# ishine/chunkformer

Hardware: AMD Instinct MI355X
Metric: audio-frames/sec (80-dim fbank) through encoder, chunkformer-large chunk=64, 1/2/4/8 GPU (higher is better)
Workload: dtype bf16

## Files before the change

chunkformer_amd/csrc/cfm_kernels.h:

```cpp
#pragma once
#include <hip/hip_runtime.h>
#include <stdint.h>

typedef __bf16 bf16;

#define CFM_HD_INLINE __host__ __device__ __forceinline__

namespace cfm {

int cu_count();

enum { EPI_STORE = 0, EPI_STORE_F32 = 1, EPI_RESID = 2, EPI_QKV = 3, EPI_GLU = 4, EPI_DW2 = 5 };
enum { ACT_NONE = 0, ACT_RELU = 1, ACT_SILU = 2, ACT_SILU_L2E = 3 };

struct EpiArgs {
  const float* bias = nullptr;
  float alpha = 1.f;
  void* out = nullptr;
  void* out2 = nullptr;
  int ldo = 0;
  int row_off = 0;
  float* x = nullptr;
  int ldx = 0;
  const uint8_t* rowmask = nullptr;
  int d = 0;
  int dk = 64;
  int col_group = 0;
  int store_mode = 0;
  int diag = 0;
  int wst = 1;
  int small_tiles = 0;
  int big_min_tiles = 0;
  int wsp_small_div = 1;
  int wsp_small_rows = 32768;
  int f16 = 0;
  const float* dw_w = nullptr;
  const float* dw_b = nullptr;
  int t2n = 0, t3n = 0;
};

int gemm_bf16_wst(int epi, int act, const bf16* A, int lda, const bf16* W, int ldw, int M, int N, int K,
                  const EpiArgs& ep, hipStream_t st);

enum { SITE_QKV = 1, SITE_OPROJ = 2, SITE_PW2 = 4, SITE_FFN2 = 8, SITE_FFN1 = 16, SITE_PW1 = 32, SITE_FE = 64 };

struct Tuning {
  int gemm_diag = 0, gemm_wst = 1, store_mode = 0, col_group = 0;
  int attn_reuse = 1;
  int conv_dot2 = 2;
  int conv_dma = 1;
  int dw2_seg = 4;
  int fe_conv = 6;
  int fe_fuse_dw2 = 1;
  int attn128_var = 1;
  int nt_sites = 8;
  int big_min_tiles = 0;
  int wsp_small_div = 1;
  int wsp_small_rows = 32768;
  int attn_min_chunks = 2;
  void apply(EpiArgs& e, int site = 0) const {
    e.diag = gemm_diag;
    e.big_min_tiles = big_min_tiles;
    e.wsp_small_div = wsp_small_div;
    e.wsp_small_rows = wsp_small_rows;
    e.wst = gemm_wst;
    e.store_mode = (nt_sites & site) ? 2 : store_mode;
    e.col_group = col_group;
  }
};

template <typename T>
int gemm(int epi, int act, const T* A, int lda, const T* W, int ldw, int M, int N, int K, const EpiArgs& ep,
         hipStream_t st);


template <typename T> struct ResidAdd {
  const T* y = nullptr;
  float alpha = 1.f;
  const uint8_t* ymask = nullptr;
  const T* y2 = nullptr;
  float alpha2 = 1.f;
  const uint8_t* ymask2 = nullptr;
  bool defer = false;
};
template <typename T>
int layernorm(float* x, const ResidAdd<T>& ra, int M, int d, const float* w, const float* b, float eps, T* out,
              const uint8_t* rowmask, hipStream_t st);
template <typename T>
int layernorm2(float* x, const ResidAdd<T>& ra, int M, int d, const float* w1, const float* b1, const float* w2,
               const float* b2, float eps, T* out, hipStream_t st);
template <typename T>
int layernorm2_f32(float* x, const ResidAdd<T>& ra, int M, int d, const float* w1, const float* b1, const float* w2,
                   const float* b2, float eps, float* out, hipStream_t st);

template <typename T>
int chunk_attention(const T* q, const T* kv, int kv_rows, const T* P, int p_rows, const float* pos_u,
                    const float* pos_v, const int32_t* desc, int nblk, int H, int dk, T* out, hipStream_t st,
                    int p_ld = 0);

CFM_HD_INLINE int qkv_kv_col(int cc, int which, int dk) { return (cc / dk) * 2 * dk + which * dk + (cc & (dk - 1)); }

int full_attention_bf16(const bf16* q, const bf16* kv, int kv_rows, const bf16* P, int p_rows, const float* pos_u,
                        const float* pos_v, const int32_t* desc, int nutt, int nd, int H, int dk, int t_keys,
                        bf16* out, hipStream_t st, int p_ld);
int chunk_attention_masked_bf16(const bf16* q, const bf16* kv, int kv_rows, const bf16* P, int p_rows,
                                const float* pos_u, const float* pos_v, const int32_t* desc, int n_chunks, int H,
                                int C, int W, bf16* out, hipStream_t st, int diag = 0, int p_ld = 0, int reuse = 1,
                                int min_chunks = 2);
int chunk_attention_masked_f16(const f16* q, const f16* kv, int kv_rows, const f16* P, int p_rows,
                               const float* pos_u, const float* pos_v, const int32_t* desc, int n_chunks, int H,
                               int C, int W, f16* out, hipStream_t st, int diag = 0, int p_ld = 0, int reuse = 1,
                               int min_chunks = 2);

bool attention_a128_eligible(int C, int W, int p_rows, int dk);
int vt_transpose_bf16(const bf16* kv, int kv_rows, int H, bf16* vt, int vt_ld, hipStream_t st);
int chunk_attention_masked_a128(const bf16* q, const bf16* kv, int kv_rows, const bf16* vt, int vt_ld, const bf16* P,
                                int p_rows, int p_ld, const float* pos_u, const float* pos_v, const int32_t* desc,
                                int n_chunks, int H, int C, int W, bf16* out, hipStream_t st, int var = 1);

template <typename T>
int conv_dw_ln_silu(const T* glu, const int32_t* desc, int nblk, int d, const float* wdw_t ,
                    const float* bdw, const float* lnw, const float* lnb, float eps, T* out, hipStream_t st,
                    int dot2 = 1, int dma = 1);

template <typename T>
int frontend_conv0_dw(const float* feats, const float* const* tab, int step, const int32_t* meta, int meta_stride,
                      int nwin, int W,
                      const float* cmvn_mean, const float* cmvn_istd, const float* w0, const float* b0,
                      const float* w1, const float* b1, const float* wpack, const float* wfrag, int d, T* out,
                      hipStream_t st, int var = 1);
constexpr int FE_WPACK = 24;
constexpr int FE2_NFRAG = 23;
template <typename T>
int frontend_dw2(const T* in, int nwin, int T2, int d, const float* w, const float* b, T* out, hipStream_t st,
                 int seg = 4);

template <typename T>
int pos_table(int d, int p_rows, int anchor, T* out, hipStream_t st);
template <typename T>
int att_cache_in(const float* cache, int L, int row_elems, T* kv, hipStream_t st);
template <typename T>
int att_cache_out(const T* kv, int start_row, int L, int row_elems, float* cache, hipStream_t st);
template <typename T>
int att_cache_in_hl(const float* cache , int H, int L, int dk, T* kv, hipStream_t st);
template <typename T>
int att_cache_out_hl(const T* kv, int start_row, int H, int L, int dk, float* cache , hipStream_t st);
template <typename T>
int cnn_cache_in(const float* cache , int d, int lorder, T* glu, hipStream_t st);
template <typename T>
int cnn_cache_out(const T* glu, int start_row, int d, int lorder, float* cache, hipStream_t st);
template <typename T>
int cache_io(bool in, bool hl, float* acache, int H, int L, int dk, T* kv, float* ccache, int d, int lorder, T* glu,
             hipStream_t st);
int masks_from_plan(const int32_t* meta, int n, int C, int L, int R, uint8_t* att, uint8_t* pad, hipStream_t st);
bool ctc_argmax_eligible(int V, int d);
int ctc_argmax_bf16(const float* enc, int M, const bf16* W, const float* bias, int V, int d, int32_t* ids,
// ... 10 lines not shown
```

chunkformer_amd/csrc/conv_module.hip:

```cpp
#include <algorithm>
#include <cstdlib>
#include <type_traits>
#include "cfm_common.h"
#include "cfm_kernels.h"

namespace cfm {

template <typename T, int VPL> struct VecIO;
template <int VPL> struct VecIO<float, VPL> {
  static CFM_DEV void load(const float* p, float (&v)[VPL]) {
#pragma unroll
    for (int e = 0; e < VPL; e += 2) {
      typedef float f2 __attribute__((ext_vector_type(2)));
      const f2 t = *reinterpret_cast<const f2*>(p + e);
      v[e] = t[0]; v[e + 1] = t[1];
    }
  }
  static CFM_DEV void store(float* p, const float (&v)[VPL]) {
#pragma unroll
    for (int e = 0; e < VPL; e += 2) {
      typedef float f2 __attribute__((ext_vector_type(2)));
      *reinterpret_cast<f2*>(p + e) = (f2){v[e], v[e + 1]};
    }
  }
// ... 110 lines not shown
#pragma unroll
  for (int r = 0; r < RW; ++r) {
    if (i0 + r >= nout) break;
    float sum = 0.f;
#pragma unroll
    for (int e = 0; e < VPL; ++e) sum += acc[r][e];
    const float mean = wave_sum(sum) / d;
    float q = 0.f;
#pragma unroll
    for (int e = 0; e < VPL; ++e) { const float t = acc[r][e] - mean; q += t * t; }
    const float rstd = rsqrtf(wave_sum(q) / d + eps);
    bvec o;
#pragma unroll
    for (int e = 0; e < VPL; ++e) o[e] = (bf16)silu_f((acc[r][e] - mean) * rstd * lw[e] + lb[e]);
    *reinterpret_cast<bvec*>(out + (size_t)(out_row0 + i0 + r) * d + c0) = o;
  }
}

typedef __bf16 bf16x2_t __attribute__((ext_vector_type(2)));
typedef _Float16 f16x2_t __attribute__((ext_vector_type(2)));
template <typename E>
CFM_DEV float dot2e(unsigned a, unsigned b, float c) {
  if constexpr (std::is_same<E, f16>::value)
    return __builtin_amdgcn_fdot2(__builtin_bit_cast(f16x2_t, a), __builtin_bit_cast(f16x2_t, b), c, false);
  else
    return __builtin_amdgcn_fdot2_f32_bf16(__builtin_bit_cast(bf16x2_t, a), __builtin_bit_cast(bf16x2_t, b), c, false);
}
template <typename E>
CFM_DEV unsigned pke(float lo, float hi) {
  typedef E e2 __attribute__((ext_vector_type(2)));
  return __builtin_bit_cast(unsigned, (e2){(E)lo, (E)hi});
}
template <int VPL, typename E>
CFM_DEV void conv_dot2_rows(const E* __restrict__ win, int nout, int out_row0, const float* __restrict__ wdw,
                            const float* __restrict__ bdw, const float* __restrict__ lnw,
                            const float* __restrict__ lnb, float eps, E* __restrict__ out, int w, int lane,
                            int win_row0 = 0) {
  constexpr int d = VPL * 64, NW = VPL / 2;
  constexpr int RW = 8;
  typedef E bvec __attribute__((ext_vector_type(VPL)));
  const int i0 = w * RW;
  if (i0 >= nout) return;
  win -= (size_t)win_row0 * d;
  const int c0 = lane * VPL;
  unsigned wp[8][VPL];
#pragma unroll
  for (int p = 0; p < 8; ++p) {
    float lo[VPL], hi[VPL];
    VecIO<float, VPL>::load(wdw + (2 * p) * d + c0, lo);
    if (p < 7) {
      VecIO<float, VPL>::load(wdw + (2 * p + 1) * d + c0, hi);
    } else {
#pragma unroll
      for (int e = 0; e < VPL; ++e) hi[e] = 0.f;
    }
#pragma unroll
    for (int e = 0; e < VPL; ++e) wp[p][e] = pke<E>(lo[e], hi[e]);
  }
  float acc[RW][VPL];
#pragma unroll
  for (int e = 0; e < VPL; ++e) {
    const float bv = bdw[c0 + e];
#pragma unroll
    for (int r = 0; r < RW; ++r) acc[r][e] = bv;
  }
  auto ld = [&](unsigned (&x)[NW], int row) {
    const unsigned* p = reinterpret_cast<const unsigned*>(win + row * d + c0);
    if constexpr (NW == 4) {
      const u32x4 t = *reinterpret_cast<const u32x4*>(p);
      x[0] = t[0]; x[1] = t[1]; x[2] = t[2]; x[3] = t[3];
    } else if constexpr (NW == 2) {
      typedef unsigned u32x2_ __attribute__((ext_vector_type(2)));
      const u32x2_ t = *reinterpret_cast<const u32x2_*>(p);
      x[0] = t[0]; x[1] = t[1];
    } else {
      x[0] = p[0];
    }
  };
  unsigned ra[NW], rb[NW];
  ld(ra, i0);
#pragma unroll
  for (int j = 0; j < RW + 14; ++j) {
    ld(rb, i0 + j + 1);
    unsigned pk[VPL];
#pragma unroll
    for (int k = 0; k < NW; ++k) {
      pk[2 * k] = __builtin_amdgcn_perm(rb[k], ra[k], 0x05040100u);
      pk[2 * k + 1] = __builtin_amdgcn_perm(rb[k], ra[k], 0x07060302u);
    }
#pragma unroll
    for (int r = 0; r < RW; ++r) {
      const int t = j - r;
      if (t >= 0 && t <= 14 && (t & 1) == 0) {
#pragma unroll
        for (int e = 0; e < VPL; ++e) acc[r][e] = dot2e<E>(pk[e], wp[t >> 1][e], acc[r][e]);
      }
    }
#pragma unroll
    for (int k = 0; k < NW; ++k) ra[k] = rb[k];
  }
  float lw[VPL], lb[VPL];
#pragma unroll
  for (int e = 0; e < VPL; ++e) {
    lw[e] = lnw[c0 + e];
    lb[e] = lnb[c0 + e];
  }
#pragma unroll
  for (int r = 0; r < RW; ++r) {
    if (i0 + r >= nout) break;
    float sum = 0.f;
#pragma unroll
    for (int e = 0; e < VPL; ++e) sum += acc[r][e];
    const float mean = wave_sum_dpp(sum) / d;
    float q = 0.f;
#pragma unroll
    for (int e = 0; e < VPL; ++e) { const float t = acc[r][e] - mean; q += t * t; }
    const float rstd = rsqrtf(wave_sum_dpp(q) / d + eps);
    bvec o;
#pragma unroll
    for (int e = 0; e < VPL; ++e) {
      const float y = (acc[r][e] - mean) * rstd * lw[e] + lb[e];
      o[e] = (E)(y * __builtin_amdgcn_rcpf(1.0f + __builtin_amdgcn_exp2f(-1.4426950408889634f * y)));
    }
    __builtin_nontemporal_store(o, reinterpret_cast<bvec*>(out + (size_t)(out_row0 + i0 + r) * d + c0));
  }
}

template <int VPL, typename E>
__global__ __launch_bounds__(512) void conv_dw_ln_silu_dot2_kernel(const E* __restrict__ glu,
                                                                   const int32_t* __restrict__ desc,
                                                                   const float* __restrict__ wdw,
                                                                   const float* __restrict__ bdw,
                                                                   const float* __restrict__ lnw,
                                                                   const float* __restrict__ lnb, float eps,
                                                                   E* __restrict__ out, int dma) {
  constexpr int d = VPL * 64, NW = VPL / 2;
  constexpr int MAXJ = 64 + 15;
  constexpr int RW = 8;
  typedef E bvec __attribute__((ext_vector_type(VPL)));
  __shared__ __attribute__((aligned(16))) E win[MAXJ * d];
  const int tid = threadIdx.x, lane = tid & 63, w = tid >> 6;
  const int32_t* D = desc + (size_t)blockIdx.x * CD_INTS;
  const int out_row0 = D[CD_OUT_ROW0], nout = D[CD_NOUT], src0 = D[CD_SRC_ROW0];
  const int nj = nout + 14;
  const int jlo = max(D[CD_J_LO], 0), jhi = min(D[CD_J_HI], nj);
  constexpr int V8 = d / 8;
  if (VPL == 8 && dma) {
    for (int j = __builtin_amdgcn_readfirstlane(w); j < MAXJ; j += 8) {
      if (j >= jlo && j < jhi)
        __builtin_amdgcn_global_load_lds((const __attribute__((address_space(1))) void*)(glu + (size_t)(src0 + j) * d + lane * 8),
                                         (__attribute__((address_space(3))) void*)(win + j * d), 16, 0, 0);
      else
        *reinterpret_cast<u32x4*>(win + j * d + lane * 8) = (u32x4){0u, 0u, 0u, 0u};
    }
    asm volatile("s_waitcnt vmcnt(0)" ::: "memory");
  } else {
    for (int idx = tid; idx < MAXJ * V8; idx += 512) {
      const int j = idx / V8, v = idx % V8;
// ... 19 lines not shown
  constexpr int HJ = QR + 15;
  __shared__ __attribute__((aligned(16))) E win[HJ * d];
  const int tid = threadIdx.x, lane = tid & 63, w = tid >> 6;
  const int half = blockIdx.y;
  const int32_t* D = desc + (size_t)blockIdx.x * CD_INTS;
  const int out_row0 = D[CD_OUT_ROW0], nout = D[CD_NOUT], src0 = D[CD_SRC_ROW0];
  if (QR * half >= nout) return;
  const int nj = nout + 14;
  const int jlo = max(D[CD_J_LO], 0), jhi = min(D[CD_J_HI], nj);
  const int r0 = QR * half;
  if (VPL == 8) {
    for (int jj = __builtin_amdgcn_readfirstlane(w); jj < HJ; jj += NWV) {
      const int j = r0 + jj;
      if (j >= jlo && j < jhi)
        __builtin_amdgcn_global_load_lds((const __attribute__((address_space(1))) void*)(glu + (size_t)(src0 + j) * d + lane * 8),
                                         (__attribute__((address_space(3))) void*)(win + jj * d), 16, 0, 0);
      else
        *reinterpret_cast<u32x4*>(win + jj * d + lane * 8) = (u32x4){0u, 0u, 0u, 0u};
    }
    asm volatile("s_waitcnt vmcnt(0)" ::: "memory");
  } else {
    constexpr int V8 = d / 8;
    for (int idx = tid; idx < HJ * V8; idx += QR * 8) {
      const int jj = idx / V8, v = idx % V8, j = r0 + jj;
      u32x4 val = (u32x4){0u, 0u, 0u, 0u};
      if (j >= jlo && j < jhi) val = *reinterpret_cast<const u32x4*>(glu + (size_t)(src0 + j) * d + v * 8);
      *reinterpret_cast<u32x4*>(win + jj * d + v * 8) = val;
    }
  }
  __syncthreads();
  conv_dot2_rows<VPL, E>(win, nout, out_row0, wdw, bdw, lnw, lnb, eps, out, NWV * half + w, lane, r0);
}

template <typename T>
int conv_dw_ln_silu(const T* glu, const int32_t* desc, int nblk, int d, const float* wdw_t, const float* bdw,
                    const float* lnw, const float* lnb, float eps, T* out, hipStream_t st, int dot2, int dma) {
  if (nblk <= 0) return 0;
  if constexpr (sizeof(T) == 2) {
    if (dot2 >= 2 && d == 512) {
      if (dot2 == 3)
        hipLaunchKernelGGL((conv_dw_ln_silu_dot2h_kernel<8, 16, T>), dim3(nblk, 4), dim3(128), 0, st, glu, desc, wdw_t, bdw, lnw, lnb, eps, out);
      else
        hipLaunchKernelGGL((conv_dw_ln_silu_dot2h_kernel<8, 32, T>), dim3(nblk, 2), dim3(256), 0, st, glu, desc, wdw_t, bdw, lnw, lnb, eps, out);
      CFM_CHECK_LAUNCH();
      return 0;
    }
    if (dot2) {
      if (d == 128) hipLaunchKernelGGL((conv_dw_ln_silu_dot2_kernel<2, T>), dim3(nblk), dim3(512), 0, st, glu, desc, wdw_t, bdw, lnw, lnb, eps, out, dma);
      else if (d == 256) hipLaunchKernelGGL((conv_dw_ln_silu_dot2_kernel<4, T>), dim3(nblk), dim3(512), 0, st, glu, desc, wdw_t, bdw, lnw, lnb, eps, out, dma);
      else if (d == 512) hipLaunchKernelGGL((conv_dw_ln_silu_dot2_kernel<8, T>), dim3(nblk), dim3(512), 0, st, glu, desc, wdw_t, bdw, lnw, lnb, eps, out, dma);
      else return (int)hipErrorInvalidValue;
      CFM_CHECK_LAUNCH();
      return 0;
    }
    if constexpr (std::is_same<T, bf16>::value) {
      if (d == 128) hipLaunchKernelGGL((conv_dw_ln_silu_lds_kernel<2>), dim3(nblk), dim3(512), 0, st, glu, desc, wdw_t, bdw, lnw, lnb, eps, out);
      else if (d == 256) hipLaunchKernelGGL((conv_dw_ln_silu_lds_kernel<4>), dim3(nblk), dim3(512), 0, st, glu, desc, wdw_t, bdw, lnw, lnb, eps, out);
      else if (d == 512) hipLaunchKernelGGL((conv_dw_ln_silu_lds_kernel<8>), dim3(nblk), dim3(512), 0, st, glu, desc, wdw_t, bdw, lnw, lnb, eps, out);
      else return (int)hipErrorInvalidValue;
      CFM_CHECK_LAUNCH();
      return 0;
    }
  }
  const dim3 grid(nblk, 4);
  if (d == 128) hipLaunchKernelGGL((conv_dw_ln_silu_kernel<T, 2>), grid, dim3(256), 0, st, glu, desc, wdw_t, bdw, lnw, lnb, eps, out);
  else if (d == 256) hipLaunchKernelGGL((conv_dw_ln_silu_kernel<T, 4>), grid, dim3(256), 0, st, glu, desc, wdw_t, bdw, lnw, lnb, eps, out);
  else if (d == 512) hipLaunchKernelGGL((conv_dw_ln_silu_kernel<T, 8>), grid, dim3(256), 0, st, glu, desc, wdw_t, bdw, lnw, lnb, eps, out);
  else return (int)hipErrorInvalidValue;
  CFM_CHECK_LAUNCH();
  return 0;
}

template int conv_dw_ln_silu<float>(const float*, const int32_t*, int, int, const float*, const float*, const float*,
                                    const float*, float, float*, hipStream_t, int, int);
template int conv_dw_ln_silu<bf16>(const bf16*, const int32_t*, int, int, const float*, const float*, const float*,
                                   const float*, float, bf16*, hipStream_t, int, int);
template int conv_dw_ln_silu<f16>(const f16*, const int32_t*, int, int, const float*, const float*, const float*,
                                   const float*, float, f16*, hipStream_t, int, int);

}
```

chunkformer_amd/csrc/model.hip:

```cpp
#include <algorithm>
#include <cmath>
#include <cstdlib>
#include <cstring>
#include <map>
#include <memory>
#include <string>
#include <vector>

#include "../../include/cfm.h"
#include "../../include/cfm_ops.h"
#include "cfm_common.h"
#include "cfm_kernels.h"
#include "plan.h"
#include "status.h"

namespace cfm {

static thread_local std::string g_err;
cfm_status set_error(cfm_status s, const std::string& msg) {
  g_err = msg;
  return s;
}

#define HIPC(x)                                                                               \
// ... 354 lines not shown
                                            tune.attn_reuse, tune.attn_min_chunks);
          else if (w.vt) {
            KCHK(vt_transpose_bf16(w.kv, kv_rows, H, w.vt, w.vt_ld, st));
            r = chunk_attention_masked_a128(w.q, w.kv, kv_rows, w.vt, w.vt_ld, w.P + (size_t)l * d, p_rows, p_ld,
                                            Lw.pu, Lw.pv, attd, aB, H, C, hh[PH_L] + C + hh[PH_R], w.ao, st,
                                            tune.attn128_var);
          }
          else if (!masked && !stream && hh[PH_L] == 0 && hh[PH_R] == 0 && hh[PH_C] == hh[PH_TOUT] &&
                   use_ring_attention && natt == hh[PH_NWIN] * ((hh[PH_TOUT] + 63) / 64))
            r = full_attention_bf16(w.q, w.kv, kv_rows, w.P + (size_t)l * d, p_rows, Lw.pu, Lw.pv, attd, hh[PH_NWIN],
                                    (hh[PH_TOUT] + 63) / 64, H, dk, hh[PH_TOUT], w.ao, st, p_ld);
        }
        if constexpr (std::is_same<T, f16>::value) {
          if (masked && use_ring_attention && dk == 64)
            r = chunk_attention_masked_f16(w.q, w.kv, kv_rows, w.P + (size_t)l * d, p_rows, Lw.pu, Lw.pv, attd, aB, H, C,
                                           hh[PH_L] + C + hh[PH_R], w.ao, st, attn_diag, p_ld, tune.attn_reuse,
                                           tune.attn_min_chunks);
        }
        if (r == -1)
          r = chunk_attention<T>(w.q, w.kv, kv_rows, w.P + (size_t)l * d, p_rows, Lw.pu, Lw.pv, attd, aB,
                                 H, dk, w.ao, st, p_ld);
        KCHK(r);
        prof_end(PC_ATTN, st, pb_);
      }
      { EpiArgs e = E(SITE_OPROJ); e.bias = Lw.b_o; e.out = w.y2; e.ldo = d;
        PROF(PC_OPROJ, gemm<T>(EPI_STORE, ACT_NONE, w.ao, d, (const T*)Lw.wo, d, rB, d, d, e, st)); }
      PROF(PC_LN, layernorm<T>(w.x, resid2(w.y, 0.5f, nullptr, w.y2, 1.f, nullptr), rB, d, Lw.ln_conv_w, Lw.ln_conv_b,
                               eps, w.h, (masked || stream) ? nullptr : rmask, st));
      if (cci && !cfuse_in) PROF(PC_CACHE, cnn_cache_in<T>(cci + l * cnn_ls, d, 7, w.glu, st));
      { EpiArgs e = E(SITE_PW1); e.bias = Lw.b_pw1; e.out = w.glu; e.ldo = d; e.row_off = gluoff;
        PROF(PC_PW1, gemm<T>(EPI_GLU, kSiluPre<T> ? ACT_SILU_L2E : ACT_NONE, w.h, d, (const T*)Lw.pw1, d, rB, 2 * d, d, e, st)); }
      if (cci && cco && !cfuse_out) PROF(PC_CACHE, cnn_cache_out<T>(w.glu, cache_start, d, 7, cco + l * cnn_ls, st));
      PROF(PC_CONV, conv_dw_ln_silu<T>(w.glu, convd, vN, d, Lw.dw_t, Lw.b_dw, Lw.cn_w, Lw.cn_b, eps, w.cv, st,
                                        tune.conv_dot2, tune.conv_dma));
      { EpiArgs e = E(SITE_PW2); e.bias = Lw.b_pw2; e.out = w.y; e.ldo = d;
        PROF(PC_PW2, gemm<T>(EPI_STORE, ACT_NONE, w.cv, d, (const T*)Lw.pw2, d, rN, d, d, e, st)); }
      { ResidAdd<T> r = resid(w.y, 1.f, rmask); r.defer = true;
        PROF(PC_LN, layernorm<T>(w.x, r, rN, d, Lw.ln_ff_w, Lw.ln_ff_b, eps, w.h, nullptr, st)); }
      { const cfm_status fs = ffn(Lw.ff1, Lw.b_ff1, Lw.ff2, Lw.b_ff2, w.y2, rN); if (fs != CFM_OK) return fs; }
      const ResidAdd<T> rf = resid2(w.y, 1.f, rmask, w.y2, 0.5f, nullptr);
      if (l + 1 < nl)
        PROF(PC_LN, layernorm2<T>(w.x, rf, rN, d, Lw.ln_fin_w, Lw.ln_fin_b, layers[l + 1].ln_ffm_w,
                                  layers[l + 1].ln_ffm_b, eps, w.h, st));
      else
        PROF(PC_LN, layernorm2_f32<T>(w.x, rf, rN, d, Lw.ln_fin_w, Lw.ln_fin_b, fe.an_w, fe.an_b, eps, out, st));
      { const cfm_status cs = caches_out(l); if (cs != CFM_OK) return cs; }
    }
    return CFM_OK;
  }

  cfm_status ctc(const float* enc, int rows, float* logp, int32_t* ids, void* ws, size_t wsb,
                 hipStream_t st) const override {
    if (!fe.ctc_w) return set_error(CFM_ERR_ASSERT, "model has no CTC head (vocab == 0)");
    const int d = cfg.d_model, V = cfg.vocab;
    if constexpr (sizeof(T) == 2) {
      if (!logp && ids && fused_ctc_ok()) {
        int r;
        if constexpr (std::is_same<T, bf16>::value)
          PROF(PC_CTC, (r = ctc_argmax_bf16(enc, rows, (const bf16*)fe.ctc_w, fe.ctc_b, V, d, ids, st)) < 0 ? 0 : r);
        else
          PROF(PC_CTC, (r = ctc_argmax_f16(enc, rows, (const f16*)fe.ctc_w, fe.ctc_b, V, d, ids, st)) < 0 ? 0 : r);
        if (r == 0) return CFM_OK;
      }
    }
    if (wsb < ctc_ws_bytes(rows)) return set_error(CFM_ERR_VALUE, "ctc workspace too small");
    float* dst = nullptr;
    { const cfm_status hs = head_logits(enc, rows, logp, ws, st, &dst); if (hs != CFM_OK) return hs; }
    PROF(PC_CTC, log_softmax_rows(dst, rows, V, logp ? 1 : 0, ids, st));
    return CFM_OK;
  }

  cfm_status head_logits(const float* enc, int rows, float* logp, void* ws, hipStream_t st, float** out) const {
    const int d = cfg.d_model, V = cfg.vocab;
    Carver c(ws);
    float* logits = c.take<float>((size_t)rows * V);
    T* a = c.take<T>((size_t)rows * d);
    const T* A;
    if constexpr (sizeof(T) == 4) {
// ... 287 lines not shown
cfm_status cfm_model_create(const cfm_config* cfg, const cfm_tensor_view* weights, int32_t n, int32_t device,
                            cfm_model** out) {
  if (!cfg || !out) return set_error(CFM_ERR_VALUE, "null argument");
  *out = nullptr;
  if (cfg->input_dim != 80) return set_error(CFM_ERR_ASSERT, "front-end kernel supports input_dim == 80");
  if (cfg->d_model != 128 && cfg->d_model != 256 && cfg->d_model != 512)
    return set_error(CFM_ERR_ASSERT, "d_model must be 128, 256 or 512");
  if (cfg->n_heads <= 0 || (cfg->d_model != 64 * cfg->n_heads && cfg->d_model != 128 * cfg->n_heads))
    return set_error(CFM_ERR_ASSERT, "head_dim (d_model / attention_heads) must be 64 or 128");
  if (cfg->ffn_dim % 128) return set_error(CFM_ERR_ASSERT, "ffn_dim must be a multiple of 128");
  if (cfg->kernel_size != 15) return set_error(CFM_ERR_ASSERT, "cnn_module_kernel must be 15");
  if (cfg->num_blocks <= 0 || cfg->vocab < 0) return set_error(CFM_ERR_VALUE, "bad num_blocks / vocab");
  HostW hw;
  for (int i = 0; i < n; ++i) hw.m[weights[i].name] = {weights[i].data, weights[i].numel};
  if (cfg->compute_dtype == CFM_DTYPE_F32) return build_model<float>(*cfg, hw, device, out);
  if (cfg->compute_dtype == CFM_DTYPE_BF16) return build_model<bf16>(*cfg, hw, device, out);
  if (cfg->compute_dtype == CFM_DTYPE_F16) return build_model<f16>(*cfg, hw, device, out);
  return set_error(CFM_ERR_VALUE, "unknown compute dtype");
}

void cfm_model_destroy(cfm_model* m) { delete m; }

cfm_status cfm_model_set_option(cfm_model* m, const char* key, int64_t value) {
  if (!m || !key) return set_error(CFM_ERR_VALUE, "null argument");
  if (!std::strcmp(key, "max_layers")) { m->max_layers = (int)value; return CFM_OK; }
  if (!std::strcmp(key, "fe_group_windows")) { m->fe_group_windows = (int)std::max<int64_t>(0, value); return CFM_OK; }
  if (!std::strcmp(key, "profile")) { m->prof_mask = (uint32_t)value; return CFM_OK; }
  if (!std::strcmp(key, "ring_attention")) { m->use_ring_attention = value != 0; return CFM_OK; }
  if (!std::strcmp(key, "ctc_fused")) { m->use_fused_ctc = value != 0; return CFM_OK; }
  {
    const std::pair<const char*, int*> knobs[] = {
        {"gemm_diag", &m->tune.gemm_diag}, {"gemm_wst", &m->tune.gemm_wst},   {"store_mode", &m->tune.store_mode},
        {"col_group", &m->tune.col_group}, {"attn_reuse", &m->tune.attn_reuse}, {"conv_dot2", &m->tune.conv_dot2},
        {"conv_dma", &m->tune.conv_dma},   {"dw2_seg", &m->tune.dw2_seg},   {"nt_sites", &m->tune.nt_sites},
        {"fe_fuse_dw2", &m->tune.fe_fuse_dw2}, {"fe_conv", &m->tune.fe_conv},
        {"attn128_var", &m->tune.attn128_var},
        {"gemm_big_min", &m->tune.big_min_tiles}, {"wsp_small_div", &m->tune.wsp_small_div},
        {"wsp_small_rows", &m->tune.wsp_small_rows},
        {"attn_min_chunks", &m->tune.attn_min_chunks}};
    for (auto& k : knobs)
      if (!std::strcmp(key, k.first)) { *k.second = (int)value; return CFM_OK; }
  }
  if (!std::strcmp(key, "attn_diag")) { m->attn_diag = (int)value; return CFM_OK; }
  if (!std::strcmp(key, "cache_fuse")) { m->cache_fuse = (int)(value != 0); return CFM_OK; }
  if (!std::strcmp(key, "trim_right")) { m->trim_right = (int)(value != 0); return CFM_OK; }
  if (!std::strcmp(key, "fe_carry")) { m->fe_carry = reinterpret_cast<float*>((intptr_t)value); return CFM_OK; }
  if (!std::strcmp(key, "fe_reuse")) { m->fe_reuse = (int)std::max<int64_t>(0, value); return CFM_OK; }
  if (!std::strcmp(key, "fe_save_from")) { m->fe_save_from = (int)value; return CFM_OK; }
  if (!std::strcmp(key, "profile_reset")) {
    m->prof_collect();
    for (int i = 0; i < PC_N; ++i) { m->prof_ms[i] = 0; m->prof_n[i] = 0; }
    return CFM_OK;
  }
  return set_error(CFM_ERR_VALUE, std::string("unknown option ") + key);
}

size_t cfm_workspace_bytes_masked(const cfm_model* m, int32_t N, int32_t C, int32_t L, int32_t R) {
  if (!m || N <= 0 || C <= 0) return 0;
  int32_t h[PH_HEADER] = {0};
  const int rows = N * C;
  h[PH_KIND] = 1; h[PH_NWIN] = N; h[PH_ROWS] = rows; h[PH_C] = C; h[PH_L] = L; h[PH_R] = R;
  h[PH_W] = (C - 1) * 8 + 15; h[PH_TOUT] = C; h[PH_PROWS] = L + 2 * C + R - 1;
  h[PH_KVROWS] = L + rows + R; h[PH_GLUROWS] = rows + 14;
  return m->ws_bytes(h);
}

// ... 224 lines not shown
```

chunkformer_amd/csrc/norm.hip:

```cpp
#include "cfm_common.h"
#include "cfm_kernels.h"

#ifndef LN_RPW
#define LN_RPW 1
#endif
#ifndef LN2_RPW
#define LN2_RPW 2
#endif
#ifndef LN_Y16
#define LN_Y16 0
#endif

namespace cfm {

template <int VPL>
CFM_DEV void ln_row(float (&v)[VPL], int d, const float* w, const float* b, float eps, int lane) {
  float s = 0.f;
#pragma unroll
  for (int e = 0; e < VPL; ++e) s += v[e];
  const float mean = wave_sum_dpp(s) / d;
  float q = 0.f;
#pragma unroll
  for (int e = 0; e < VPL; ++e) {
    const float t = v[e] - mean;
// ... 116 lines not shown
      }
    }
    ln_row<VPL>(v0, d, w, b, eps, lane);
    ln_row<VPL>(v1, d, w, b, eps, lane);
    if (rowmask) {
#pragma unroll
      for (int e = 0; e < VPL; ++e) {
        if (!rowmask[row0]) v0[e] = 0.f;
        if (!rowmask[row1]) v1[e] = 0.f;
      }
    }
    store_row(out + (size_t)row0 * d + lane * VPL, v0);
    if (row1 != row0) store_row(out + (size_t)row1 * d + lane * VPL, v1);
    return;
  }
  const int row = blockIdx.x * 4 + (threadIdx.x >> 6);
  if (row >= M) return;
  float v[VPL];
  float* xp = x + (size_t)row * d + lane * VPL;
  load_row(xp, v);
  resid_add<T, VPL>(v, xp, ra, row, lane);
  ln_row<VPL>(v, d, w, b, eps, lane);
  if (rowmask && !rowmask[row]) {
#pragma unroll
    for (int e = 0; e < VPL; ++e) v[e] = 0.f;
  }
  store_row(out + (size_t)row * d + lane * VPL, v);
}

template <typename TY, typename TO, int VPL>
__global__ __launch_bounds__(256) void ln2_kernel(float* __restrict__ x, ResidAdd<TY> ra, int M,
                                                  const float* __restrict__ w1, const float* __restrict__ b1,
                                                  const float* __restrict__ w2, const float* __restrict__ b2, float eps,
                                                  TO* __restrict__ out) {
  const int lane = threadIdx.x & 63;
  constexpr int d = VPL * 64;
  if constexpr (LN2_RPW == 2) {
    const int row0 = (blockIdx.x * 4 + (threadIdx.x >> 6)) * 2;
    if (row0 >= M) return;
    const int row1 = row0 + 1 < M ? row0 + 1 : row0;
    float v0[VPL], v1[VPL];
    float* xp0 = x + (size_t)row0 * d + lane * VPL;
    float* xp1 = x + (size_t)row1 * d + lane * VPL;
    load_row(xp0, v0);
    load_row(xp1, v1);
    if (ra.y) {
      resid_terms<TY, VPL>(v0, ra, row0, lane);
      resid_terms<TY, VPL>(v1, ra, row1, lane);
    }
    ln_row<VPL>(v0, d, w1, b1, eps, lane);
    ln_row<VPL>(v1, d, w1, b1, eps, lane);
    store_row(xp0, v0);
    if (row1 != row0) store_row(xp1, v1);
    if (w2) {
      ln_row<VPL>(v0, d, w2, b2, eps, lane);
      ln_row<VPL>(v1, d, w2, b2, eps, lane);
    }
    store_row(out + (size_t)row0 * d + lane * VPL, v0);
    if (row1 != row0) store_row(out + (size_t)row1 * d + lane * VPL, v1);
    return;
  }
  const int row = blockIdx.x * 4 + (threadIdx.x >> 6);
  if (row >= M) return;
  float v[VPL];
  float* xp = x + (size_t)row * d + lane * VPL;
  load_row(xp, v);
  if (ra.y) resid_terms<TY, VPL>(v, ra, row, lane);
  ln_row<VPL>(v, d, w1, b1, eps, lane);
  store_row(xp, v);
  if (w2) ln_row<VPL>(v, d, w2, b2, eps, lane);
  store_row(out + (size_t)row * d + lane * VPL, v);
}

template <typename T>
int layernorm(float* x, const ResidAdd<T>& ra, int M, int d, const float* w, const float* b, float eps, T* out,
              const uint8_t* rowmask, hipStream_t st) {
  if (M <= 0) return 0;
  const int nblk = (M + 4 * LN_RPW - 1) / (4 * LN_RPW);
  if (d == 128) hipLaunchKernelGGL((ln_kernel<T, 2>), dim3(nblk), dim3(256), 0, st, x, ra, M, w, b, eps, out, rowmask);
  else if (d == 256) hipLaunchKernelGGL((ln_kernel<T, 4>), dim3(nblk), dim3(256), 0, st, x, ra, M, w, b, eps, out, rowmask);
  else if (d == 512) hipLaunchKernelGGL((ln_kernel<T, 8>), dim3(nblk), dim3(256), 0, st, x, ra, M, w, b, eps, out, rowmask);
  else return (int)hipErrorInvalidValue;
  CFM_CHECK_LAUNCH();
  return 0;
}

template <typename TY, typename TO>
static int ln2_launch(float* x, const ResidAdd<TY>& ra, int M, int d, const float* w1, const float* b1, const float* w2,
                      const float* b2, float eps, TO* out, hipStream_t st) {
  if (M <= 0) return 0;
  const int nblk = (M + 4 * LN2_RPW - 1) / (4 * LN2_RPW);
  if (d == 128) hipLaunchKernelGGL((ln2_kernel<TY, TO, 2>), dim3(nblk), dim3(256), 0, st, x, ra, M, w1, b1, w2, b2, eps, out);
  else if (d == 256) hipLaunchKernelGGL((ln2_kernel<TY, TO, 4>), dim3(nblk), dim3(256), 0, st, x, ra, M, w1, b1, w2, b2, eps, out);
  else if (d == 512) hipLaunchKernelGGL((ln2_kernel<TY, TO, 8>), dim3(nblk), dim3(256), 0, st, x, ra, M, w1, b1, w2, b2, eps, out);
  else return (int)hipErrorInvalidValue;
  CFM_CHECK_LAUNCH();
  return 0;
}

template <typename T>
int layernorm2(float* x, const ResidAdd<T>& ra, int M, int d, const float* w1, const float* b1, const float* w2,
               const float* b2, float eps, T* out, hipStream_t st) {
  return ln2_launch<T, T>(x, ra, M, d, w1, b1, w2, b2, eps, out, st);
}
template <typename T>
int layernorm2_f32(float* x, const ResidAdd<T>& ra, int M, int d, const float* w1, const float* b1, const float* w2,
                   const float* b2, float eps, float* out, hipStream_t st) {
  return ln2_launch<T, float>(x, ra, M, d, w1, b1, w2, b2, eps, out, st);
}

template int layernorm<float>(float*, const ResidAdd<float>&, int, int, const float*, const float*, float, float*,
                              const uint8_t*, hipStream_t);
template int layernorm<bf16>(float*, const ResidAdd<bf16>&, int, int, const float*, const float*, float, bf16*,
                             const uint8_t*, hipStream_t);
template int layernorm<f16>(float*, const ResidAdd<f16>&, int, int, const float*, const float*, float, f16*,
                             const uint8_t*, hipStream_t);
template int layernorm2<float>(float*, const ResidAdd<float>&, int, int, const float*, const float*, const float*,
                               const float*, float, float*, hipStream_t);
template int layernorm2<bf16>(float*, const ResidAdd<bf16>&, int, int, const float*, const float*, const float*,
                              const float*, float, bf16*, hipStream_t);
template int layernorm2<f16>(float*, const ResidAdd<f16>&, int, int, const float*, const float*, const float*,
                              const float*, float, f16*, hipStream_t);
template int layernorm2_f32<float>(float*, const ResidAdd<float>&, int, int, const float*, const float*, const float*,
                                   const float*, float, float*, hipStream_t);
template int layernorm2_f32<bf16>(float*, const ResidAdd<bf16>&, int, int, const float*, const float*, const float*,
                                  const float*, float, float*, hipStream_t);
template int layernorm2_f32<f16>(float*, const ResidAdd<f16>&, int, int, const float*, const float*, const float*,
                                  const float*, float, float*, hipStream_t);

}
```

Measured before the change: 32.68 million.

## Add persistent double-buffered conv kernel and skip final-layer residual store

Adds a persistent depthwise-conv+LN+SiLU kernel that walks chunk groups per CU with double-buffered LDS staging through global_load_lds, and reuses overlapping halo rows between consecutive chunks. It is selected only when conv_dot2==4, and the default is 2, so it is opt-in through a new conv_blocks knob. Separately, the last layer's layernorm2_f32 now skips writing the normalized residual back to x, which saves one full-width fp32 store that nothing downstream reads. The LN change is on by default, and it is a problem if any later consumer does read x after the final layer.

```diff
diff --git a/chunkformer_amd/csrc/cfm_kernels.h b/chunkformer_amd/csrc/cfm_kernels.h
--- a/chunkformer_amd/csrc/cfm_kernels.h
+++ b/chunkformer_amd/csrc/cfm_kernels.h
@@ -48,6 +48,7 @@
   int gemm_diag = 0, gemm_wst = 1, store_mode = 0, col_group = 0;
   int attn_reuse = 1;
   int conv_dot2 = 2;
+  int conv_blocks = 0;
   int conv_dma = 1;
   int dw2_seg = 4;
   int fe_conv = 6;
@@ -91,7 +92,7 @@
                const float* b2, float eps, T* out, hipStream_t st);
 template <typename T>
 int layernorm2_f32(float* x, const ResidAdd<T>& ra, int M, int d, const float* w1, const float* b1, const float* w2,
-                   const float* b2, float eps, float* out, hipStream_t st);
+                   const float* b2, float eps, float* out, hipStream_t st, bool store_x = true);
 
 template <typename T>
 int chunk_attention(const T* q, const T* kv, int kv_rows, const T* P, int p_rows, const float* pos_u,
@@ -121,7 +122,7 @@
 template <typename T>
 int conv_dw_ln_silu(const T* glu, const int32_t* desc, int nblk, int d, const float* wdw_t ,
                     const float* bdw, const float* lnw, const float* lnb, float eps, T* out, hipStream_t st,
-                    int dot2 = 1, int dma = 1);
+                    int dot2 = 1, int dma = 1, int blocks = 0);
 
 template <typename T>
 int frontend_conv0_dw(const float* feats, const float* const* tab, int step, const int32_t* meta, int meta_stride,
diff --git a/chunkformer_amd/csrc/conv_module.hip b/chunkformer_amd/csrc/conv_module.hip
--- a/chunkformer_amd/csrc/conv_module.hip
+++ b/chunkformer_amd/csrc/conv_module.hip
@@ -166,18 +166,8 @@
   return __builtin_bit_cast(unsigned, (e2){(E)lo, (E)hi});
 }
 template <int VPL, typename E>
-CFM_DEV void conv_dot2_rows(const E* __restrict__ win, int nout, int out_row0, const float* __restrict__ wdw,
-                            const float* __restrict__ bdw, const float* __restrict__ lnw,
-                            const float* __restrict__ lnb, float eps, E* __restrict__ out, int w, int lane,
-                            int win_row0 = 0) {
-  constexpr int d = VPL * 64, NW = VPL / 2;
-  constexpr int RW = 8;
-  typedef E bvec __attribute__((ext_vector_type(VPL)));
-  const int i0 = w * RW;
-  if (i0 >= nout) return;
-  win -= (size_t)win_row0 * d;
-  const int c0 = lane * VPL;
-  unsigned wp[8][VPL];
+CFM_DEV void conv_dot2_taps(const float* __restrict__ wdw, int c0, unsigned (&wp)[8][VPL]) {
+  constexpr int d = VPL * 64;
 #pragma unroll
   for (int p = 0; p < 8; ++p) {
     float lo[VPL], hi[VPL];
@@ -191,10 +181,15 @@
 #pragma unroll
     for (int e = 0; e < VPL; ++e) wp[p][e] = pke<E>(lo[e], hi[e]);
   }
-  float acc[RW][VPL];
+}
+template <int VPL, typename E>
+CFM_DEV void conv_dot2_acc(const E* __restrict__ win, int i0, int c0, const unsigned (&wp)[8][VPL],
+                           const float (&bias)[VPL], float (&acc)[8][VPL]) {
+  constexpr int d = VPL * 64, NW = VPL / 2;
+  constexpr int RW = 8;
 #pragma unroll
   for (int e = 0; e < VPL; ++e) {
-    const float bv = bdw[c0 + e];
+    const float bv = bias[e];
 #pragma unroll
     for (int r = 0; r < RW; ++r) acc[r][e] = bv;
   }
@@ -233,31 +228,61 @@
 #pragma unroll
     for (int k = 0; k < NW; ++k) ra[k] = rb[k];
   }
+}
+template <int VPL, typename E, bool STORE = true>
+CFM_DEV void conv_dot2_finish(float (&acc)[8][VPL], const float (&lw)[VPL], const float (&lb)[VPL], float eps,
+                              int nout, int i0, int out_row0, int c0, E* __restrict__ out) {
+  constexpr int d = VPL * 64;
+  constexpr int RW = 8;
+  typedef E bvec __attribute__((ext_vector_type(VPL)));
+#pragma unroll
+  for (int r = 0; r < RW; ++r) {
+    if (i0 + r >= nout) break;
+    float sum = 0.f;
+#pragma unroll
+    for (int e = 0; e < VPL; ++e) sum += acc[r][e];
+    const float mean = wave_sum_dpp(sum) / d;
+    float q = 0.f;
+#pragma unroll
+    for (int e = 0; e < VPL; ++e) { const float t = acc[r][e] - mean; q += t * t; }
+    const float rstd = rsqrtf(wave_sum_dpp(q) / d + eps);
+    bvec o;
+#pragma unroll
+    for (int e = 0; e < VPL; ++e) {
+      const float y = (acc[r][e] - mean) * rstd * lw[e] + lb[e];
+      o[e] = (E)(y * __builtin_amdgcn_rcpf(1.0f + __builtin_amdgcn_exp2f(-1.4426950408889634f * y)));
+    }
+    if constexpr (STORE)
+      __builtin_nontemporal_store(o, reinterpret_cast<bvec*>(out + (size_t)(out_row0 + i0 + r) * d + c0));
+    else if (o[0] == (E)12345.f)
+      __builtin_nontemporal_store(o, reinterpret_cast<bvec*>(out + (size_t)(out_row0 + i0 + r) * d + c0));
+  }
+}
+template <int VPL, typename E>
+CFM_DEV void conv_dot2_rows(const E* __restrict__ win, int nout, int out_row0, const float* __restrict__ wdw,
+                            const float* __restrict__ bdw, const float* __restrict__ lnw,
+                            const float* __restrict__ lnb, float eps, E* __restrict__ out, int w, int lane,
+                            int win_row0 = 0) {
+  constexpr int d = VPL * 64;
+  constexpr int RW = 8;
+  const int i0 = w * RW;
+  if (i0 >= nout) return;
+  win -= (size_t)win_row0 * d;
+  const int c0 = lane * VPL;
+  unsigned wp[8][VPL];
+  conv_dot2_taps<VPL, E>(wdw, c0, wp);
+  float bias[VPL];
+#pragma unroll
+  for (int e = 0; e < VPL; ++e) bias[e] = bdw[c0 + e];
+  float acc[RW][VPL];
+  conv_dot2_acc<VPL, E>(win, i0, c0, wp, bias, acc);
   float lw[VPL], lb[VPL];
 #pragma unroll
   for (int e = 0; e < VPL; ++e) {
     lw[e] = lnw[c0 + e];
     lb[e] = lnb[c0 + e];
   }
-#pragma unroll
-  for (int r = 0; r < RW; ++r) {
-    if (i0 + r >= nout) break;
-    float sum = 0.f;
-#pragma unroll
-    for (int e = 0; e < VPL; ++e) sum += acc[r][e];
-    const float mean = wave_sum_dpp(sum) / d;
-    float q = 0.f;
-#pragma unroll
-    for (int e = 0; e < VPL; ++e) { const float t = acc[r][e] - mean; q += t * t; }
-    const float rstd = rsqrtf(wave_sum_dpp(q) / d + eps);
-    bvec o;
-#pragma unroll
-    for (int e = 0; e < VPL; ++e) {
-      const float y = (acc[r][e] - mean) * rstd * lw[e] + lb[e];
-      o[e] = (E)(y * __builtin_amdgcn_rcpf(1.0f + __builtin_amdgcn_exp2f(-1.4426950408889634f * y)));
-    }
-    __builtin_nontemporal_store(o, reinterpret_cast<bvec*>(out + (size_t)(out_row0 + i0 + r) * d + c0));
-  }
+  conv_dot2_finish<VPL, E>(acc, lw, lb, eps, nout, i0, out_row0, c0, out);
 }
 
 template <int VPL, typename E>
@@ -343,11 +368,138 @@
   conv_dot2_rows<VPL, E>(win, nout, out_row0, wdw, bdw, lnw, lnb, eps, out, NWV * half + w, lane, r0);
 }
 
+#ifndef CFM_CONV_DIAG
+#define CFM_CONV_DIAG 0
+#endif
+template <typename E>
+__global__ __launch_bounds__(512) void conv_dw_ln_silu_dot2p_kernel(const E* __restrict__ glu,
+                                                                    const int32_t* __restrict__ desc, int nblk,
+                                                                    const float* __restrict__ wdw,
+                                                                    const float* __restrict__ bdw,
+                                                                    const float* __restrict__ lnw,
+                                                                    const float* __restrict__ lnb, float eps,
+                                                                    E* __restrict__ out) {
+  constexpr int VPL = 8, d = 512;
+  constexpr int WJ = 64 + 15;
+  __shared__ __attribute__((aligned(16))) E win[2][WJ * d];
+  const int lane = threadIdx.x & 63, w = __builtin_amdgcn_readfirstlane(threadIdx.x >> 6);
+  const long long G = 8ll * nblk;
+  const int g0 = (int)(G * blockIdx.x / gridDim.x), g1 = (int)(G * (blockIdx.x + 1) / gridDim.x);
+  if (g0 >= g1) return;
+  const int c0 = lane * VPL;
+  unsigned wp[8][VPL];
+  conv_dot2_taps<VPL, E>(wdw, c0, wp);
+  float bias[VPL], lw[VPL], lb[VPL];
+#pragma unroll
+  for (int e = 0; e < VPL; ++e) {
+    bias[e] = bdw[c0 + e];
+    lw[e] = lnw[c0 + e];
+    lb[e] = lnb[c0 + e];
+  }
+  struct It { int out_row0, nout, src0, jlo, jhi, ga, ng; };
+  auto fetch = [&](int s) {
+    const int32_t* D = desc + (size_t)(s >> 3) * CD_INTS;
+    It c;
+    c.out_row0 = D[CD_OUT_ROW0]; c.nout = D[CD_NOUT]; c.src0 = D[CD_SRC_ROW0];
+    c.jlo = max(D[CD_J_LO], 0); c.jhi = min(D[CD_J_HI], c.nout + 14);
+    c.ga = s & 7; c.ng = min(8 - c.ga, g1 - s);
+    return c;
+  };
+  auto stage = [&](const It& c, E* dst, bool cont, const E* prv) {
+    const int hi = 8 * (c.ga + c.ng) + 15;
+    for (int j = 8 * c.ga + w; j < hi; j += 8) {
+      const bool real = j >= c.jlo && j < c.jhi;
+      if (real && !(cont && j < 14)) {
+        __builtin_amdgcn_global_load_lds((const __attribute__((address_space(1))) void*)(glu + (size_t)(c.src0 + j) * d + lane * 8),
+                                         (__attribute__((address_space(3))) void*)(dst + j * d), 16, 0, 0);
+      } else {
+        u32x4 v = (u32x4){0u, 0u, 0u, 0u};
+        if (real) v = *reinterpret_cast<const u32x4*>(prv + (64 + j) * d + lane * 8);
+        *reinterpret_cast<u32x4*>(dst + j * d + lane * 8) = v;
+      }
+    }
+  };
+  auto continues = [](const It& p, const It& c) {
+    return c.ga == 0 && p.ga + p.ng == 8 && c.src0 == p.src0 + 64 && p.jlo <= 64 && p.jhi >= 78;
+  };
+  int s = g0, pb = 0;
+  It cur = fetch(s), nxt = cur;
+  s += cur.ng;
+  stage(cur, win[0], false, win[0]);
+  asm volatile("s_waitcnt vmcnt(0)" ::: "memory");
+  __syncthreads();
+  bool has_nxt = s < g1;
+  if (has_nxt) {
+    nxt = fetch(s);
+    s += nxt.ng;
+    stage(nxt, win[1], continues(cur, nxt), win[0]);
+  }
+  for (;;) {
+    const int i0 = 8 * (cur.ga + w);
+    const bool act = w < cur.ng && i0 < cur.nout;
+    float acc[8][VPL];
+    if (act) {
+      if constexpr (CFM_CONV_DIAG == 3 || CFM_CONV_DIAG == 5) {
+#pragma unroll
+        for (int r = 0; r < 8; ++r)
+#pragma unroll
+          for (int e = 0; e < VPL; ++e) acc[r][e] = bias[e];
+      } else {
+        conv_dot2_acc<VPL, E>(win[pb], i0, c0, wp, bias, acc);
+      }
+    }
+    if (has_nxt) {
+      if constexpr (CFM_CONV_DIAG == 1) {
+        asm volatile("s_waitcnt lgkmcnt(0)\n\ts_barrier" ::: "memory");
+      } else {
+        asm volatile("s_waitcnt vmcnt(0)" ::: "memory");
+        __syncthreads();
+      }
+    }
+    It nn = nxt;
+    const bool has_nn = has_nxt && s < g1;
+    if (has_nn) {
+      nn = fetch(s);
+      s += nn.ng;
+      stage(nn, win[pb], continues(nxt, nn), win[pb ^ 1]);
+    }
+    if (act) {
+      if constexpr (CFM_CONV_DIAG == 4 || CFM_CONV_DIAG == 5) {
+        typedef E bvec __attribute__((ext_vector_type(VPL)));
+#pragma unroll
+        for (int r = 0; r < 8; ++r) {
+          bvec o;
+#pragma unroll
+          for (int e = 0; e < VPL; ++e) o[e] = (E)acc[r][e];
+          if (i0 + r < cur.nout)
+            __builtin_nontemporal_store(o, reinterpret_cast<bvec*>(out + (size_t)(cur.out_row0 + i0 + r) * d + c0));
+        }
+      } else {
+        conv_dot2_finish<VPL, E, CFM_CONV_DIAG != 2>(acc, lw, lb, eps, cur.nout, i0, cur.out_row0, c0, out);
+      }
+    }
+    if (!has_nxt) break;
+    cur = nxt; nxt = nn; has_nxt = has_nn; pb ^= 1;
+  }
+  if constexpr (CFM_CONV_DIAG == 1) asm volatile("s_waitcnt vmcnt(0)" ::: "memory");
+}
+
+constexpr int CONV_PERSIST_MIN = 4;
+
 template <typename T>
 int conv_dw_ln_silu(const T* glu, const int32_t* desc, int nblk, int d, const float* wdw_t, const float* bdw,
-                    const float* lnw, const float* lnb, float eps, T* out, hipStream_t st, int dot2, int dma) {
+                    const float* lnw, const float* lnb, float eps, T* out, hipStream_t st, int dot2, int dma,
+                    int blocks) {
   if (nblk <= 0) return 0;
   if constexpr (sizeof(T) == 2) {
+    if (dot2 == 4 && d == 512) {
+      const int grid = blocks > 0 ? std::min(blocks, cu_count()) : cu_count();
+      if (blocks > 0 || nblk >= CONV_PERSIST_MIN * grid) {
+        hipLaunchKernelGGL((conv_dw_ln_silu_dot2p_kernel<T>), dim3(grid), dim3(512), 0, st, glu, desc, nblk, wdw_t, bdw, lnw, lnb, eps, out);
+        CFM_CHECK_LAUNCH();
+        return 0;
+      }
+    }
     if (dot2 >= 2 && d == 512) {
       if (dot2 == 3)
         hipLaunchKernelGGL((conv_dw_ln_silu_dot2h_kernel<8, 16, T>), dim3(nblk, 4), dim3(128), 0, st, glu, desc, wdw_t, bdw, lnw, lnb, eps, out);
@@ -383,10 +535,10 @@
 }
 
 template int conv_dw_ln_silu<float>(const float*, const int32_t*, int, int, const float*, const float*, const float*,
-                                    const float*, float, float*, hipStream_t, int, int);
+                                    const float*, float, float*, hipStream_t, int, int, int);
 template int conv_dw_ln_silu<bf16>(const bf16*, const int32_t*, int, int, const float*, const float*, const float*,
-                                   const float*, float, bf16*, hipStream_t, int, int);
+                                   const float*, float, bf16*, hipStream_t, int, int, int);
 template int conv_dw_ln_silu<f16>(const f16*, const int32_t*, int, int, const float*, const float*, const float*,
-                                   const float*, float, f16*, hipStream_t, int, int);
-
-}
+                                   const float*, float, f16*, hipStream_t, int, int, int);
+
+}
diff --git a/chunkformer_amd/csrc/model.hip b/chunkformer_amd/csrc/model.hip
--- a/chunkformer_amd/csrc/model.hip
+++ b/chunkformer_amd/csrc/model.hip
@@ -410,7 +410,7 @@
         PROF(PC_PW1, gemm<T>(EPI_GLU, kSiluPre<T> ? ACT_SILU_L2E : ACT_NONE, w.h, d, (const T*)Lw.pw1, d, rB, 2 * d, d, e, st)); }
       if (cci && cco && !cfuse_out) PROF(PC_CACHE, cnn_cache_out<T>(w.glu, cache_start, d, 7, cco + l * cnn_ls, st));
       PROF(PC_CONV, conv_dw_ln_silu<T>(w.glu, convd, vN, d, Lw.dw_t, Lw.b_dw, Lw.cn_w, Lw.cn_b, eps, w.cv, st,
-                                        tune.conv_dot2, tune.conv_dma));
+                                        tune.conv_dot2, tune.conv_dma, tune.conv_blocks));
       { EpiArgs e = E(SITE_PW2); e.bias = Lw.b_pw2; e.out = w.y; e.ldo = d;
         PROF(PC_PW2, gemm<T>(EPI_STORE, ACT_NONE, w.cv, d, (const T*)Lw.pw2, d, rN, d, d, e, st)); }
       { ResidAdd<T> r = resid(w.y, 1.f, rmask); r.defer = true;
@@ -421,7 +421,7 @@
         PROF(PC_LN, layernorm2<T>(w.x, rf, rN, d, Lw.ln_fin_w, Lw.ln_fin_b, layers[l + 1].ln_ffm_w,
                                   layers[l + 1].ln_ffm_b, eps, w.h, st));
       else
-        PROF(PC_LN, layernorm2_f32<T>(w.x, rf, rN, d, Lw.ln_fin_w, Lw.ln_fin_b, fe.an_w, fe.an_b, eps, out, st));
+        PROF(PC_LN, layernorm2_f32<T>(w.x, rf, rN, d, Lw.ln_fin_w, Lw.ln_fin_b, fe.an_w, fe.an_b, eps, out, st, false));
       { const cfm_status cs = caches_out(l); if (cs != CFM_OK) return cs; }
     }
     return CFM_OK;
@@ -775,6 +775,7 @@
     const std::pair<const char*, int*> knobs[] = {
         {"gemm_diag", &m->tune.gemm_diag}, {"gemm_wst", &m->tune.gemm_wst},   {"store_mode", &m->tune.store_mode},
         {"col_group", &m->tune.col_group}, {"attn_reuse", &m->tune.attn_reuse}, {"conv_dot2", &m->tune.conv_dot2},
+        {"conv_blocks", &m->tune.conv_blocks},
         {"conv_dma", &m->tune.conv_dma},   {"dw2_seg", &m->tune.dw2_seg},   {"nt_sites", &m->tune.nt_sites},
         {"fe_fuse_dw2", &m->tune.fe_fuse_dw2}, {"fe_conv", &m->tune.fe_conv},
         {"attn128_var", &m->tune.attn128_var},
diff --git a/chunkformer_amd/csrc/norm.hip b/chunkformer_amd/csrc/norm.hip
--- a/chunkformer_amd/csrc/norm.hip
+++ b/chunkformer_amd/csrc/norm.hip
@@ -172,7 +172,7 @@
 __global__ __launch_bounds__(256) void ln2_kernel(float* __restrict__ x, ResidAdd<TY> ra, int M,
                                                   const float* __restrict__ w1, const float* __restrict__ b1,
                                                   const float* __restrict__ w2, const float* __restrict__ b2, float eps,
-                                                  TO* __restrict__ out) {
+                                                  TO* __restrict__ out, bool store_x) {
   const int lane = threadIdx.x & 63;
   constexpr int d = VPL * 64;
   if constexpr (LN2_RPW == 2) {
@@ -190,8 +190,10 @@
     }
     ln_row<VPL>(v0, d, w1, b1, eps, lane);
     ln_row<VPL>(v1, d, w1, b1, eps, lane);
-    store_row(xp0, v0);
-    if (row1 != row0) store_row(xp1, v1);
+    if (store_x) {
+      store_row(xp0, v0);
+      if (row1 != row0) store_row(xp1, v1);
+    }
     if (w2) {
       ln_row<VPL>(v0, d, w2, b2, eps, lane);
       ln_row<VPL>(v1, d, w2, b2, eps, lane);
@@ -207,7 +209,7 @@
   load_row(xp, v);
   if (ra.y) resid_terms<TY, VPL>(v, ra, row, lane);
   ln_row<VPL>(v, d, w1, b1, eps, lane);
-  store_row(xp, v);
+  if (store_x) store_row(xp, v);
   if (w2) ln_row<VPL>(v, d, w2, b2, eps, lane);
   store_row(out + (size_t)row * d + lane * VPL, v);
 }
@@ -227,12 +229,12 @@
 
 template <typename TY, typename TO>
 static int ln2_launch(float* x, const ResidAdd<TY>& ra, int M, int d, const float* w1, const float* b1, const float* w2,
-                      const float* b2, float eps, TO* out, hipStream_t st) {
+                      const float* b2, float eps, TO* out, hipStream_t st, bool store_x = true) {
   if (M <= 0) return 0;
   const int nblk = (M + 4 * LN2_RPW - 1) / (4 * LN2_RPW);
-  if (d == 128) hipLaunchKernelGGL((ln2_kernel<TY, TO, 2>), dim3(nblk), dim3(256), 0, st, x, ra, M, w1, b1, w2, b2, eps, out);
-  else if (d == 256) hipLaunchKernelGGL((ln2_kernel<TY, TO, 4>), dim3(nblk), dim3(256), 0, st, x, ra, M, w1, b1, w2, b2, eps, out);
-  else if (d == 512) hipLaunchKernelGGL((ln2_kernel<TY, TO, 8>), dim3(nblk), dim3(256), 0, st, x, ra, M, w1, b1, w2, b2, eps, out);
+  if (d == 128) hipLaunchKernelGGL((ln2_kernel<TY, TO, 2>), dim3(nblk), dim3(256), 0, st, x, ra, M, w1, b1, w2, b2, eps, out, store_x);
+  else if (d == 256) hipLaunchKernelGGL((ln2_kernel<TY, TO, 4>), dim3(nblk), dim3(256), 0, st, x, ra, M, w1, b1, w2, b2, eps, out, store_x);
+  else if (d == 512) hipLaunchKernelGGL((ln2_kernel<TY, TO, 8>), dim3(nblk), dim3(256), 0, st, x, ra, M, w1, b1, w2, b2, eps, out, store_x);
   else return (int)hipErrorInvalidValue;
   CFM_CHECK_LAUNCH();
   return 0;
@@ -245,8 +247,8 @@
 }
 template <typename T>
 int layernorm2_f32(float* x, const ResidAdd<T>& ra, int M, int d, const float* w1, const float* b1, const float* w2,
-                   const float* b2, float eps, float* out, hipStream_t st) {
-  return ln2_launch<T, float>(x, ra, M, d, w1, b1, w2, b2, eps, out, st);
+                   const float* b2, float eps, float* out, hipStream_t st, bool store_x) {
+  return ln2_launch<T, float>(x, ra, M, d, w1, b1, w2, b2, eps, out, st, store_x);
 }
 
 template int layernorm<float>(float*, const ResidAdd<float>&, int, int, const float*, const float*, float, float*,
@@ -262,10 +264,10 @@
 template int layernorm2<f16>(float*, const ResidAdd<f16>&, int, int, const float*, const float*, const float*,
                               const float*, float, f16*, hipStream_t);
 template int layernorm2_f32<float>(float*, const ResidAdd<float>&, int, int, const float*, const float*, const float*,
-                                   const float*, float, float*, hipStream_t);
+                                   const float*, float, float*, hipStream_t, bool);
 template int layernorm2_f32<bf16>(float*, const ResidAdd<bf16>&, int, int, const float*, const float*, const float*,
-                                  const float*, float, float*, hipStream_t);
+                                  const float*, float, float*, hipStream_t, bool);
 template int layernorm2_f32<f16>(float*, const ResidAdd<f16>&, int, int, const float*, const float*, const float*,
-                                  const float*, float, float*, hipStream_t);
-
-}
+                                  const float*, float, float*, hipStream_t, bool);
+
+}
```

Result: no change. 32.73 million, median of 6 (+0.2%).
